# FanmingL/Recurrent-Offpolicy-RL

Hardware: AMD Instinct MI355X
Metric: env-steps/sec trained (higher is better)
Workload: dtype f32; 1 GPU; smamba_s32_c16_b2_nln SAC-REDQ update, B=64/GPU, T=1024, D=256 (configs[1]; N=8: configs[3]); row_length=1043, obs=17, act=6, critic=efc-8, global_rows=64, parallelism=dp1

## Files before the change

### include/resel_hip.h

```cpp
#ifndef RESEL_HIP_H
#define RESEL_HIP_H

#include <stddef.h>
#include <stdint.h>

#ifdef __cplusplus
extern "C" {
#endif

#define RESEL_OK 0
#define RESEL_EINVAL (-1)
#define RESEL_ELAUNCH (-2)

typedef void* resel_stream_t;

int resel_abi_version(void);
const char* resel_build_info(void);

enum {
    RESEL_PROF_SSCAN_FWD = 0, RESEL_PROF_SSCAN_BWD = 1, RESEL_PROF_ATTN_FWD = 2, RESEL_PROF_ATTN_DQ = 3, RESEL_PROF_ATTN_DKV = 4,
    RESEL_PROF_LINREC_REAL_FWD = 5, RESEL_PROF_LINREC_REAL_BWD = 6, RESEL_PROF_LINREC_COMPLEX_FWD = 7, RESEL_PROF_LINREC_COMPLEX_BWD = 8,
    RESEL_PROF_GRU_FWD = 9, RESEL_PROF_GRU_BWD = 10, RESEL_PROF_CONV_FWD = 11, RESEL_PROF_CONV_BWD = 12, RESEL_PROF_GEMM = 13,
    RESEL_PROF_SSCAN_FWD_LOCAL = 14, RESEL_PROF_SSCAN_BWD_LOCAL = 15,
    RESEL_PROF_NSLOTS = 16
};
int resel_profile_enable(int on);
int resel_profile_collect(int kernel_id, double* total_us, int* launches);

#define RESEL_SSCAN_CKPT 8
size_t resel_selective_scan_ckpt_bytes(int B, int L, int Di, int N);
size_t resel_selective_scan_fwd_workspace_bytes(int B, int L, int Di, int N, int time_segments);
int resel_selective_scan_fwd(const float* u, int64_t ld_u, const float* delta, int64_t ld_delta,
                             const float* z, int64_t ld_z, const float* A,
                             const float* Bm, int64_t ld_b, const float* Cm, int64_t ld_c,
                             const float* D, const float* delta_bias, const float* start,
                             float* out, int64_t ld_out, float* ckpt, float* last_state, void* workspace,
                             int B, int L, int Di, int N, int delta_softplus, int time_segments,
                             void* amax_out, unsigned amax_epoch, resel_stream_t stream);

size_t resel_selective_scan_bwd_workspace_bytes(int B, int L, int Di, int N, int time_segments);
int resel_selective_scan_bwd(const float* u, int64_t ld_u, const float* delta, int64_t ld_delta,
                             const float* z, int64_t ld_z, const float* A,
                             const float* Bm, int64_t ld_b, const float* Cm, int64_t ld_c,
                             const float* D, const float* delta_bias, const float* start,
                             const float* dout, int64_t ld_dout, const float* ckpt,
                             float* du, int64_t ld_du, float* ddelta, int64_t ld_ddelta, float* dz, int64_t ld_dz,
                             float* dBm, int64_t ld_db, float* dCm, int64_t ld_dc,
                             float* dA, float* dD, float* ddelta_bias, void* workspace,
                             int B, int L, int Di, int N, int delta_softplus, int time_segments,
                             void* amax_dz, void* amax_ddelta, unsigned amax_epoch, resel_stream_t stream);

int resel_causal_conv1d_fwd(const float* x, int64_t ld_x, const float* w, const float* bias, const float* mask,
                            float* y, int64_t ld_y, int B, int L, int Di, int K, int silu, void* amax_y, unsigned amax_epoch,
                            resel_stream_t stream);
size_t resel_causal_conv1d_bwd_workspace_bytes(int B, int L, int Di, int K);
int resel_causal_conv1d_bwd(const float* x, int64_t ld_x, const float* w, const float* bias, const float* mask,
                            const float* dy, int64_t ld_dy, float* dx, int64_t ld_dx, float* dw, float* dbias,
                            void* workspace, int B, int L, int Di, int K, int silu, void* amax_dx, unsigned amax_epoch,
                            resel_stream_t stream);
int resel_causal_conv1d_bwd2(const float* x, int64_t ld_x, const float* w, const float* bias, const float* mask,
                             const float* dy, int64_t ld_dy, const float* dy2, int64_t ld_dy2, float* dx, int64_t ld_dx,
                             float* dw, float* dbias, void* workspace, int B, int L, int Di, int K, int silu,
                             void* amax_dx, unsigned amax_epoch, resel_stream_t stream);

int resel_add_layernorm_fwd(const float* x, const float* residual, const float* w, const float* b,
                            float* y, float* res_out, float* stats, int M, int C, float eps, int rms, int act,
                            void* amax_y, unsigned amax_epoch, resel_stream_t stream);
size_t resel_add_layernorm_bwd_workspace_bytes(int M, int C);
int resel_add_layernorm_bwd(const float* dy, const float* dres_in, const float* res, const float* w, const float* b,
                            const float* stats, float* dx, float* dw, float* db, void* workspace,
                            int M, int C, int rms, int has_bias, int act, void* amax_dx, unsigned amax_epoch, resel_stream_t stream);

int resel_linrec_real_fwd(const float* v, const float* f, int64_t ld_u, const float* start, const float* h0, float* h,
                          int B, int L, int C, int fuse_act, void* amax_h, unsigned amax_epoch, resel_stream_t stream);
int resel_linrec_real_bwd(const float* v, const float* f, int64_t ld_u, const float* start, const float* h0, const float* h,
                          const float* dh, float* dv, float* df, int64_t ld_du, int B, int L, int C, int fuse_act,
                          void* amax_du, unsigned amax_epoch, resel_stream_t stream);
int resel_linrec_complex_fwd(const float* vr, const float* vi, int64_t ld_u, const float* lam_re, const float* lam_im,
                             const float* gamma, const float* start, const float* h0r, const float* h0i,
                             float* hr, float* hi, int B, int L, int C, void* amax_h, unsigned amax_epoch, resel_stream_t stream);
size_t resel_linrec_complex_bwd_workspace_bytes(int B, int L, int C);
int resel_linrec_complex_bwd(const float* vr, const float* vi, int64_t ld_u, const float* lam_re, const float* lam_im,
                             const float* gamma, const float* start, const float* h0r, const float* h0i,
// ... 184 lines not shown
```

### recurrent-offpolicy-rl_amd/csrc/resel_common.h

```cpp
#pragma once
#include <hip/hip_runtime.h>
#include <hip/hip_ext.h>
#include <stdint.h>
#include "../../include/resel_hip.h"

#define RESEL_LOG2E 1.4426950408889634f
#define RESEL_LN2 0.6931471805599453f

namespace resel {

typedef const float __attribute__((address_space(4)))* cfloat_p;
__device__ __forceinline__ cfloat_p as_uniform(const float* p) {
    return (cfloat_p)(uintptr_t)p;
}

__device__ __forceinline__ float fast_exp2(float x) { return __builtin_amdgcn_exp2f(x); }
__device__ __forceinline__ float fast_exp(float x) { return __builtin_amdgcn_exp2f(x * RESEL_LOG2E); }
__device__ __forceinline__ float fast_rcp(float x) { return __builtin_amdgcn_rcpf(x); }

__device__ __forceinline__ float sigmoidf_(float x) { return fast_rcp(1.0f + fast_exp(-x)); }
__device__ __forceinline__ float siluf_(float x) { return x * fast_rcp(1.0f + fast_exp(-x)); }
__device__ __forceinline__ float dsiluf_(float x) {
    float s = sigmoidf_(x);
    return s * (1.0f + x * (1.0f - s));
// ... 73 lines not shown
    (void)hipEventCreate(&b);
    hipExtLaunchKernelGGL(kernel, grid, block, lds, s, a, b, 0, args...);
    prof_push(slot, a, b);
}

#define RESEL_AMAX_SUBSLOTS 8
#define RESEL_AMAX_STRIDE 16
struct AmaxOut { unsigned long long* slot; unsigned epoch; };
__device__ __forceinline__ float amax4(float m, float4 v) {
    return fmaxf(fmaxf(m, fmaxf(__builtin_fabsf(v.x), __builtin_fabsf(v.y))), fmaxf(__builtin_fabsf(v.z), __builtin_fabsf(v.w)));
}
__device__ __forceinline__ void amax_publish_wave(float m, AmaxOut o) {
    if (o.slot == nullptr) return;
#pragma unroll
    for (int s = 32; s > 0; s >>= 1) m = fmaxf(m, __shfl_xor(m, s, 64));
    if (__lane_id() == 0) {
        unsigned long long* w = o.slot + RESEL_AMAX_STRIDE * ((blockIdx.x + blockIdx.y + blockIdx.z) & (RESEL_AMAX_SUBSLOTS - 1));
        const unsigned long long mine = ((unsigned long long)o.epoch << 32) | __float_as_uint(m);
        if (*(volatile unsigned long long*)w < mine) atomicMax(w, mine);
    }
}
__device__ __forceinline__ float amax_read(const float* handle) {
    const unsigned long long* h = reinterpret_cast<const unsigned long long*>(handle);
    const int j = __lane_id() & (RESEL_AMAX_SUBSLOTS - 1);
    unsigned long long v = h[RESEL_AMAX_STRIDE * j];
#pragma unroll
    for (int s = RESEL_AMAX_SUBSLOTS / 2; s > 0; s >>= 1) {
        const unsigned long long o = __shfl_xor(v, s, 64);
        v = o > v ? o : v;
    }
    return __uint_as_float((unsigned)(v & 0xffffffffu));
}

inline int launch_status() { return hipGetLastError() == hipSuccess ? RESEL_OK : RESEL_ELAUNCH; }
const unsigned long long* dropout_offset_base();
inline bool aligned16(const void* p) { return (reinterpret_cast<uintptr_t>(p) & 15u) == 0; }

}
```

### recurrent-offpolicy-rl_amd/csrc/selective_scan.hip

```cpp
#include "resel_common.h"
#include <hip/hip_ext.h>
#include <type_traits>
#include <vector>

namespace {
using namespace resel;

template <typename K, typename P>
void launch_maybe_timed(int slot, K kernel, dim3 grid, dim3 block, hipStream_t s, const P& p) {
    launch_timed(slot, kernel, grid, block, 0, s, p);
}
#ifdef SSCAN_STAMP
unsigned long long* g_stamps = nullptr;
#endif

constexpr int TILE_C = 64;
constexpr int CKS = RESEL_SSCAN_CKPT;
constexpr int SC = 16;
constexpr int SCH = 8;
static_assert(2 * CKS == SC && CKS == SCH, "a backward sub-chunk is two checkpoint intervals: each 8-step half starts from a stored state");

struct FwdParams {
    const float *u, *delta, *z, *A, *Bm, *Cm, *D, *delta_bias, *start;
    float *out, *ckpt, *last_state;
// ... 1035 lines not shown
                                        const float* Bm, int64_t ld_b, const float* Cm, int64_t ld_c,
                                        const float* D, const float* delta_bias, const float* start,
                                        float* out, int64_t ld_out, float* ckpt, float* last_state, void* workspace,
                                        int B, int L, int Di, int N, int delta_softplus, int time_segments,
                                        void* amax_out, unsigned amax_epoch, resel_stream_t stream) {
    if (!u || !delta || !A || !Bm || !Cm || !out || B <= 0 || L <= 0 || Di <= 0) return RESEL_EINVAL;
    if (amax_out && (reinterpret_cast<uintptr_t>(amax_out) & 7u)) return RESEL_EINVAL;
    if (Di % 4 != 0 || ld_u % 4 || ld_delta % 4 || ld_out % 4 || (z && ld_z % 4)) return RESEL_EINVAL;
    if (!aligned16(u) || !aligned16(delta) || !aligned16(out) || (z && !aligned16(z))) return RESEL_EINVAL;
    if ((D && !aligned16(D)) || (delta_bias && !aligned16(delta_bias))) return RESEL_EINVAL;
    FwdParams p{u, delta, z, A, Bm, Cm, D, delta_bias, start, out, ckpt, last_state,
                ld_u, ld_delta, ld_z, ld_b, ld_c, ld_out, B, L, Di, N, n_ckpt(L), delta_softplus & 3,
                (Di + TILE_C - 1) / TILE_C,
                (ld_b % 4 == 0 && ld_c % 4 == 0 && aligned16(Bm) && aligned16(Cm)) ? 1 : 0, (delta_softplus >> 2) & 1, 0, 1, nullptr, nullptr,
                AmaxOut{(unsigned long long*)amax_out, amax_epoch}};
#ifdef SSCAN_STAMP
    p.stamps = g_stamps;
#endif
    hipStream_t s = (hipStream_t)stream;
    switch (N) {
        case 4: return launch_fwd<1, 4, 32>(p, time_segments, workspace, s);
        case 8: return launch_fwd<2, 4, 32>(p, time_segments, workspace, s);
        case 16: return launch_fwd<4, 4, 32>(p, time_segments, workspace, s);
        case 32: return launch_fwd<8, 4, 32>(p, time_segments, workspace, s);
        case 64: return launch_fwd<8, 8, 32>(p, time_segments, workspace, s);
        default: return RESEL_EINVAL;
    }
}

extern "C" size_t resel_selective_scan_bwd_workspace_bytes(int B, int L, int Di, int N, int time_segments) {
    return bwd_ws(B, L, Di, N, time_segments).total;
}

extern "C" int resel_selective_scan_bwd(const float* u, int64_t ld_u, const float* delta, int64_t ld_delta,
                                        const float* z, int64_t ld_z, const float* A,
                                        const float* Bm, int64_t ld_b, const float* Cm, int64_t ld_c,
                                        const float* D, const float* delta_bias, const float* start,
                                        const float* dout, int64_t ld_dout, const float* ckpt,
                                        float* du, int64_t ld_du, float* ddelta, int64_t ld_ddelta,
                                        float* dz, int64_t ld_dz, float* dBm, int64_t ld_db, float* dCm, int64_t ld_dc,
                                        float* dA, float* dD, float* ddelta_bias, void* workspace,
                                        int B, int L, int Di, int N, int delta_softplus, int time_segments,
                                        void* amax_dz, void* amax_ddelta, unsigned amax_epoch, resel_stream_t stream) {
    if (!u || !delta || !A || !Bm || !Cm || !dout || !du || !ddelta || !dBm || !dCm || !dA || !workspace)
        return RESEL_EINVAL;
    if ((reinterpret_cast<uintptr_t>(amax_dz) & 7u) || (reinterpret_cast<uintptr_t>(amax_ddelta) & 7u)) return RESEL_EINVAL;
    if (B <= 0 || L <= 0 || Di <= 0 || Di % 4 != 0 || N % 4 != 0) return RESEL_EINVAL;
    if ((z != nullptr) != (dz != nullptr)) return RESEL_EINVAL;
    if (n_ckpt(L) > 0 && !ckpt) return RESEL_EINVAL;
    if (ld_u % 4 || ld_delta % 4 || ld_dout % 4 || ld_du % 4 || ld_ddelta % 4 || (z && (ld_z % 4 || ld_dz % 4)))
        return RESEL_EINVAL;
    if (!aligned16(u) || !aligned16(delta) || !aligned16(dout) || !aligned16(du) || !aligned16(ddelta) ||
        (z && (!aligned16(z) || !aligned16(dz))) || (D && !aligned16(D)) || (delta_bias && !aligned16(delta_bias)) ||
        !aligned16(workspace))
        return RESEL_EINVAL;
    const BwdWs ws = bwd_ws(B, L, Di, N, time_segments);
    char* base = (char*)workspace;
    BwdParams p{u, delta, z, A, Bm, Cm, D, delta_bias, start, dout, ckpt, du, ddelta, dz,
                (float*)(base + ws.dB), (float*)(base + ws.dC), (float*)(base + ws.dA), (float*)(base + ws.dD),
                (float*)(base + ws.dbias),
                ld_u, ld_delta, ld_z, ld_b, ld_c, ld_dout, ld_du, ld_ddelta, ld_dz,
                B, L, Di, N, n_ckpt(L), delta_softplus & 3, (Di + TILE_C - 1) / TILE_C,
                (ld_b % 4 == 0 && ld_c % 4 == 0 && aligned16(Bm) && aligned16(Cm)) ? 1 : 0, (delta_softplus >> 2) & 1,
                ws.nseg > 1 ? ((L + ws.nseg - 1) / ws.nseg + 31) / 32 * 32 : L, ws.nseg,
                ws.nseg > 1 ? (float*)(base + ws.carry) : nullptr, ws.nseg > 1 ? (float*)(base + ws.sdl) : nullptr,
                AmaxOut{(unsigned long long*)amax_dz, amax_epoch}, AmaxOut{(unsigned long long*)amax_ddelta, amax_epoch}};
    hipStream_t s = (hipStream_t)stream;
    int rc;
    switch (N) {
        case 4: rc = launch_bwd<1, 4>(p, s); break;
        case 8: rc = launch_bwd<2, 4>(p, s); break;
        case 16: rc = launch_bwd<4, 4>(p, s); break;
        case 32: rc = launch_bwd<8, 4>(p, s); break;
        case 64: rc = launch_bwd<8, 8>(p, s); break;
        default: return RESEL_EINVAL;
    }
    if (rc != RESEL_OK) return rc;
    const int64_t ntok = (int64_t)B * L;
    const int64_t n4 = ntok * (N / 4);
    hipLaunchKernelGGL(sscan_reduce_bc_kernel, dim3((unsigned)((n4 + 255) / 256), 2), dim3(256), 0, s,
                       p.dB_part, p.dC_part, p.nd, ntok, N, dBm, ld_db, dCm, ld_dc);
    const int64_t na = (int64_t)Di * N;
    hipLaunchKernelGGL(sscan_param_grads_kernel, dim3((unsigned)((na + 15) / 16), 3), dim3(256), 0, s,
                       p.dA_part, p.dD_part, p.dbias_part, B * ws.nseg, (int)na, Di, A, p.a_log, dA, dD, ddelta_bias);
    return launch_status();
}
```

### recurrent-offpolicy-rl_amd/csrc/skinny_gemm.hip

```cpp
#include "resel_common.h"

namespace {
using namespace resel;

typedef float f32x16 __attribute__((ext_vector_type(16)));

__device__ __forceinline__ int acc_row(int r, int half) { return (r >> 2) * 8 + half * 4 + (r & 3); }

template <int NT>
__global__ __launch_bounds__(256) void atb_kernel(const float* __restrict__ Wm, int64_t ldw, int Wd, const float* __restrict__ Nm,
                                                  int64_t ldn, int Nd, float* __restrict__ part, int64_t K, int rows_per,
                                                  int transposed) {
    const int lane = threadIdx.x & 63, wave = threadIdx.x >> 6;
    const int half = lane >> 5, col = lane & 31;
    const int wb = blockIdx.y * 512 + wave * 128;
    if (wb >= Wd) return;
    const int64_t k0 = (int64_t)blockIdx.x * rows_per;
    const int64_t k1 = k0 + rows_per < K ? k0 + rows_per : K;
    f32x16 acc[4][NT];
#pragma unroll
    for (int e = 0; e < 4; ++e)
#pragma unroll
        for (int t = 0; t < NT; ++t)
#pragma unroll
// ... 16 lines not shown
            for (int t = 0; t < NT; ++t) b[u][t] = (ok && n_ok[t]) ? Nm[kr * ldn + 32 * t + col] : 0.f;
        }
#pragma unroll
        for (int u = 0; u < UN; ++u)
#pragma unroll
            for (int t = 0; t < NT; ++t) {
                acc[0][t] = __builtin_amdgcn_mfma_f32_32x32x2f32(a[u].x, b[u][t], acc[0][t], 0, 0, 0);
                acc[1][t] = __builtin_amdgcn_mfma_f32_32x32x2f32(a[u].y, b[u][t], acc[1][t], 0, 0, 0);
                acc[2][t] = __builtin_amdgcn_mfma_f32_32x32x2f32(a[u].z, b[u][t], acc[2][t], 0, 0, 0);
                acc[3][t] = __builtin_amdgcn_mfma_f32_32x32x2f32(a[u].w, b[u][t], acc[3][t], 0, 0, 0);
            }
    }
    float* dst = part + (int64_t)blockIdx.x * Wd * Nd;
#pragma unroll
    for (int e = 0; e < 4; ++e)
#pragma unroll
        for (int t = 0; t < NT; ++t) {
            const int n = 32 * t + col;
            if (n >= Nd) continue;
#pragma unroll
            for (int r = 0; r < 16; ++r) {
                const int w = wb + 4 * acc_row(r, half) + e;
                if (w < Wd) dst[transposed ? (int64_t)n * Wd + w : (int64_t)w * Nd + n] = acc[e][t][r];
            }
        }
}

inline int pick_ksplit(int64_t K, int Wd, int Nd) {
    int64_t ks = (int64_t)(16 << 20) / ((int64_t)Wd * Nd * 4);
    if (ks > 512) ks = 512;
    if (ks < 32) ks = 32;
    if (ks > (K + 1) / 2) ks = (K + 1) / 2;
    return (int)(ks < 1 ? 1 : ks);
}

}

extern "C" {

size_t resel_atb_workspace_bytes(int64_t K, int Wd, int Nd) {
    return (size_t)pick_ksplit(K, Wd, Nd) * Wd * Nd * sizeof(float);
}

int resel_atb(const float* wide, int64_t ldw, int Wd, const float* narrow, int64_t ldn, int Nd, float* out, int transposed,
              void* workspace, int64_t K, resel_stream_t stream) {
    if (!wide || !narrow || !out || !workspace || K <= 0 || Wd <= 0 || Nd <= 0) return RESEL_EINVAL;
    if (Nd > 96 || (Wd & 3) || (ldw & 3) || !aligned16(wide)) return RESEL_EINVAL;
    const int ks = pick_ksplit(K, Wd, Nd);
    int rows_per = (int)((K + ks - 1) / ks);
    rows_per += rows_per & 1;
    const int nsplit = (int)((K + rows_per - 1) / rows_per);
    const dim3 grid(nsplit, (Wd + 511) / 512), block(256);
    hipStream_t s = (hipStream_t)stream;
    float* part = (float*)workspace;
    const int NT = (Nd + 31) / 32;
    switch (NT) {
        case 1: hipLaunchKernelGGL(atb_kernel<1>, grid, block, 0, s, wide, ldw, Wd, narrow, ldn, Nd, part, K, rows_per, transposed); break;
        case 2: hipLaunchKernelGGL(atb_kernel<2>, grid, block, 0, s, wide, ldw, Wd, narrow, ldn, Nd, part, K, rows_per, transposed); break;
        default: hipLaunchKernelGGL(atb_kernel<3>, grid, block, 0, s, wide, ldw, Wd, narrow, ldn, Nd, part, K, rows_per, transposed); break;
    }
    launch_colsum(part, (int64_t)Wd * Nd, nsplit, Wd * Nd, out, s);
    return launch_status();
}

}
```

### recurrent-offpolicy-rl_amd/offpolicy_rnn/hip/_lib.py

```python
import ctypes
import os
from ctypes import c_float, c_int, c_int64, c_size_t, c_uint64, c_void_p

_HERE = os.path.dirname(os.path.abspath(__file__))
LIB_PATH = os.environ.get('RESEL_HIP_LIBRARY') or os.path.join(_HERE, 'libresel_hip.so')
ABI_VERSION = 11
_lib = None

P, I, L, F, S, U = c_void_p, c_int, c_int64, c_float, c_void_p, c_uint64
E = ctypes.c_uint

RESET_MAX_SEGS, RESET_MAX_COUNTERS = 16, 8


class ResetSeg(ctypes.Structure):
    _fields_ = [('base', c_void_p), ('row_stride', c_int64), ('width', ctypes.c_int32)]


class ResetSegs(ctypes.Structure):
    _fields_ = [('seg', ResetSeg * RESET_MAX_SEGS)]


class ResetCounters(ctypes.Structure):
    _fields_ = [('pos', c_void_p * RESET_MAX_COUNTERS)]


SIGNATURES = {
    'resel_abi_version': (c_int, []),
    'resel_build_info': (ctypes.c_char_p, []),
    'resel_profile_enable': (c_int, [I]),
    'resel_profile_collect': (c_int, [I, P, P]),
    'resel_selective_scan_ckpt_bytes': (c_size_t, [I, I, I, I]),
    'resel_selective_scan_fwd_workspace_bytes': (c_size_t, [I, I, I, I, I]),
    'resel_selective_scan_fwd': (c_int, [P, L, P, L, P, L, P, P, L, P, L, P, P, P, P, L, P, P, P, I, I, I, I, I, I, P, E, S]),
    'resel_selective_scan_bwd_workspace_bytes': (c_size_t, [I, I, I, I, I]),
    'resel_selective_scan_bwd': (c_int, [P, L, P, L, P, L, P, P, L, P, L, P, P, P, P, L, P,
                                         P, L, P, L, P, L, P, L, P, L, P, P, P, P, I, I, I, I, I, I, P, P, E, S]),
    'resel_causal_conv1d_fwd': (c_int, [P, L, P, P, P, P, L, I, I, I, I, I, P, E, S]),
    'resel_causal_conv1d_bwd_workspace_bytes': (c_size_t, [I, I, I, I]),
    'resel_causal_conv1d_bwd': (c_int, [P, L, P, P, P, P, L, P, L, P, P, P, I, I, I, I, I, P, E, S]),
    'resel_causal_conv1d_bwd2': (c_int, [P, L, P, P, P, P, L, P, L, P, L, P, P, P, I, I, I, I, I, P, E, S]),
    'resel_add_layernorm_fwd': (c_int, [P, P, P, P, P, P, P, I, I, F, I, I, P, E, S]),
    'resel_add_layernorm_bwd_workspace_bytes': (c_size_t, [I, I]),
    'resel_add_layernorm_bwd': (c_int, [P, P, P, P, P, P, P, P, P, P, I, I, I, I, I, P, E, S]),
    'resel_linrec_real_fwd': (c_int, [P, P, L, P, P, P, I, I, I, I, P, E, S]),
    'resel_linrec_real_bwd': (c_int, [P, P, L, P, P, P, P, P, P, L, I, I, I, I, P, E, S]),
    'resel_linrec_complex_fwd': (c_int, [P, P, L, P, P, P, P, P, P, P, P, I, I, I, P, E, S]),
    'resel_linrec_complex_bwd_workspace_bytes': (c_size_t, [I, I, I]),
    'resel_place_blocks': (c_int, [P, L, I, I, I, P, P, P, P, P, P, S]),
    'resel_lru_params_fwd': (c_int, [P, P, I, S]),
    'resel_lru_params_bwd': (c_int, [P, P, P, I, S]),
    'resel_linrec_complex_bwd': (c_int, [P, P, L, P, P, P, P, P, P, P, P, P, P, P, P, L, P, P, P, P, I, I, I, S]),
    'resel_gru_workspace_bytes': (c_size_t, [I, I, I]),
    'resel_gru_seq_fwd': (c_int, [P, P, P, P, P, P, P, I, I, I, S]),
    'resel_gru_seq_bwd': (c_int, [P, P, P, P, P, P, P, P, I, I, I, S]),
    'resel_gru_multi_workspace_bytes': (c_size_t, [I, I, I, I]),
    'resel_gru_multi_fwd': (c_int, [I, P, P, P, P, P, P, P, I, I, I, S]),
    'resel_gru_multi_form': (c_int, [I, I, I]),
    'resel_attn_varlen_fwd_workspace_bytes': (c_size_t, [I, I]),
    'resel_attn_varlen_fwd': (c_int, [P, P, P, P, P, P, I, I, I, I, I, F, F, U, U, S]),
    'resel_attn_varlen_bwd_workspace_bytes': (c_size_t, [I, I, I, I, I]),
    'resel_attn_varlen_bwd': (c_int, [P, P, P, P, P, P, P, P, I, I, I, I, I, F, F, U, U, S]),
    'resel_attn_varlen_fwd_padded': (c_int, [P, P, P, P, P, P, I, I, I, I, I, F, F, U, U, S]),
    'resel_attn_varlen_bwd_padded': (c_int, [P, P, P, P, P, P, P, P, I, I, I, I, I, F, F, U, U, S]),
    'resel_pack_rows': (c_int, [P, L, P, P, P, L, I, I, S]),
    'resel_unpack_rows': (c_int, [P, L, P, P, P, L, I, I, I, S]),
    'resel_dropout': (c_int, [P, P, L, F, U, U, S]),
    'resel_dropout_offset_base': (c_int, [P]),
    'resel_gelu_dropout_fwd': (c_int, [P, P, L, F, U, U, P, E, S]),
    'resel_gelu_dropout_bwd': (c_int, [P, P, P, L, F, U, U, P, E, S]),
# ... 82 lines not shown
```

### recurrent-offpolicy-rl_amd/offpolicy_rnn/hip/ops.py

```python
import ctypes
import os
from typing import Optional

import torch

from ._lib import check, lib


def _need_cuda(name, *ts):
    for t in ts:
        if t is not None and not t.is_cuda:
            raise RuntimeError(f'RESeL-HIP: {name} needs CUDA tensors (got a {t.device} tensor); the HIP kernels are the '
                               f'only implementation of this op - there is no CPU fallback.')


def _p(t: Optional[torch.Tensor]):
    return None if t is None else ctypes.c_void_p(t.data_ptr())


if hasattr(torch._C, '_cuda_getCurrentRawStream') and hasattr(torch._C, '_cuda_getDevice'):
    def _stream():
        return ctypes.c_void_p(torch._C._cuda_getCurrentRawStream(torch._C._cuda_getDevice()))
else:
    def _stream():
# ... 38 lines not shown
    out = {}
    for kid, name in enumerate(PROF_SLOTS):
        tot, n = ctypes.c_double(0.0), ctypes.c_int(0)
        check(lib().resel_profile_collect(kid, ctypes.byref(tot), ctypes.byref(n)), 'profile_collect')
        if n.value:
            out[name] = (n.value, tot.value / n.value)
    return out


SSCAN_TIME_SEGMENTS = int(os.environ.get('RESEL_SSCAN_TIME_SEGMENTS', '0'))


def _sscan_fwd(Bsz, L, u, delta, z, A, Bm, Cm, D, delta_bias, start, out, ck, last, softplus, amax_out=None, epoch=0):
    Di, N = A.shape
    nb = lib().resel_selective_scan_fwd_workspace_bytes(Bsz, L, Di, N, SSCAN_TIME_SEGMENTS)
    check(lib().resel_selective_scan_fwd(
        _p(u), u.stride(-2), _p(delta), delta.stride(-2), _p(z), 0 if z is None else z.stride(-2), _p(A),
        _p(Bm), Bm.stride(-2), _p(Cm), Cm.stride(-2), _p(D), _p(delta_bias), _p(start),
        _p(out), out.stride(-2), _p(ck), _p(last), _p(_ws(nb, u.device) if nb else None), Bsz, L, Di, N, softplus,
        SSCAN_TIME_SEGMENTS, amax_out, epoch, _stream()), 'selective_scan_fwd')


def _sscan_bwd(Bsz, L, u, delta, z, A, Bm, Cm, D, delta_bias, start, dout, ck, du, ddelta, dz, dB, dC, dA, dD, dbias, softplus,
               amax_dz=None, amax_ddelta=None, epoch=0):
    Di, N = A.shape
    ws = _ws(lib().resel_selective_scan_bwd_workspace_bytes(Bsz, L, Di, N, SSCAN_TIME_SEGMENTS), u.device)
    check(lib().resel_selective_scan_bwd(
        _p(u), u.stride(-2), _p(delta), delta.stride(-2), _p(z), 0 if z is None else z.stride(-2), _p(A),
        _p(Bm), Bm.stride(-2), _p(Cm), Cm.stride(-2), _p(D), _p(delta_bias), _p(start),
        _p(dout), dout.stride(-2), _p(ck),
        _p(du), du.stride(-2), _p(ddelta), ddelta.stride(-2), _p(dz), 0 if dz is None else dz.stride(-2),
        _p(dB), dB.stride(-2), _p(dC), dC.stride(-2), _p(dA), _p(dD), _p(dbias), _p(ws),
        Bsz, L, Di, N, softplus, SSCAN_TIME_SEGMENTS, amax_dz, amax_ddelta, epoch, _stream()), 'selective_scan_bwd')


def _conv_fwd(Bsz, L, x, w, bias, mask, y, act, amax_y=None, epoch=0):
    Di, K = w.shape
    check(lib().resel_causal_conv1d_fwd(_p(x), x.stride(-2), _p(w), _p(bias), _p(mask), _p(y), y.stride(-2), Bsz, L, Di, K, act,
                                        amax_y, epoch, _stream()), 'causal_conv1d_fwd')


def _conv_bwd(Bsz, L, x, w, bias, mask, dy, dy2, dx, dw, db, act, amax_dx=None, epoch=0):
    Di, K = w.shape
    ws = _ws(lib().resel_causal_conv1d_bwd_workspace_bytes(Bsz, L, Di, K), x.device)
    check(lib().resel_causal_conv1d_bwd2(_p(x), x.stride(-2), _p(w), _p(bias), _p(mask), _p(dy), dy.stride(-2),
                                         _p(dy2), 0 if dy2 is None else dy2.stride(-2), _p(dx), dx.stride(-2), _p(dw), _p(db), _p(ws),
                                         Bsz, L, Di, K, act, amax_dx, epoch, _stream()), 'causal_conv1d_bwd')


class SelectiveScanFn(torch.autograd.Function):

    @staticmethod
    def forward(ctx, u, delta, A, Bm, Cm, D, z, delta_bias, start, delta_softplus, return_last_state):
        _need_cuda('selective_scan', u, delta, A, Bm, Cm)
        u, delta, Bm, Cm = _tok_major(u), _tok_major(delta), _tok_major(Bm), _tok_major(Cm)
        z = None if z is None else _tok_major(z)
        A = A.float().contiguous()
        D = None if D is None else D.float().contiguous()
        delta_bias = None if delta_bias is None else delta_bias.float().contiguous()
        Bsz, L, Di = u.shape
        N = A.shape[1]
        start = _flags(start, Bsz, L)
        out = torch.empty(Bsz, L, Di, dtype=torch.float32, device=u.device)
        need_grad = any(ctx.needs_input_grad)
        ck = None
        if need_grad:
# ... 73 lines not shown
        need_grad = any(ctx.needs_input_grad)
        ck = _ws(lib().resel_selective_scan_ckpt_bytes(Bsz, L, Di, N), x.device) if need_grad else None
        y = torch.empty(M, Di, dtype=torch.float32, device=x.device)
        h_y, p_y, e_y = _slot_args(track, x.device)
        _sscan_fwd(Bsz, L, xc, dt, xz[:, Di:], A, x_dbl[:, R:R + N], x_dbl[:, R + N:], D, None, startf, y, ck, None, 6, p_y, e_y)
        tag_amax(y, h_y)
        out = mm_nt(y, out_w)
        ctx.handles = keep_handles(ctx.ax, h_xc, h_y)
        ctx.save_for_backward(x2, in_w, cw, conv_b, xproj_w, dt_w, dt_b, A, D, out_w, maskf, startf, xz, xc, x_dbl, dt, y, ck)
        ctx.dims = (Bsz, L, Dm, Di, N, R, K, conv_w.shape)
        return out.view(Bsz, L, -1)

    @staticmethod
    def backward(ctx, dout):
        (x2, in_w, cw, conv_b, xproj_w, dt_w, dt_b, A, D, out_w, maskf, startf, xz, xc, x_dbl, dt, y, ck) = ctx.saved_tensors
        Bsz, L, Dm, Di, N, R, K, cw_shape = ctx.dims
        M = Bsz * L
        dev = x2.device
        do2 = dout.reshape(M, -1)
        if not do2.is_contiguous():
            do2 = do2.contiguous()
        ax, h_xc, h_y = live_handles(ctx.handles)
        d_out_w = wgrad(do2, y, amax_x=h_y)
        dy = mm_nn(do2, out_w)
        dxz = torch.empty(M, 2 * Di, dtype=torch.float32, device=dev)
        dx_dbl = torch.empty(M, R + 2 * N, dtype=torch.float32, device=dev)
        dxc = torch.empty(M, Di, dtype=torch.float32, device=dev)
        ddt = torch.empty(M, Di, dtype=torch.float32, device=dev)
        dA = torch.empty(Di, N, dtype=torch.float32, device=dev)
        dD = torch.empty(Di, dtype=torch.float32, device=dev)
        ddt_b = torch.empty(Di, dtype=torch.float32, device=dev)
        track = amax_tracking() and M * Di >= (1 << 20)
        h_dxz, p_dxz, e_b = _slot_args(track, dev)
        h_ddt, p_ddt, _ = _slot_args(track, dev)
        _sscan_bwd(Bsz, L, xc, dt, xz[:, Di:], A, x_dbl[:, R:R + N], x_dbl[:, R + N:], D, None, startf, dy, ck,
                   dxc, ddt, dxz[:, Di:], dx_dbl[:, R:R + N], dx_dbl[:, R + N:], dA, dD, ddt_b, 6, p_dxz, p_ddt, e_b)
        tag_amax(ddt, h_ddt)
        d_dt_w = atb(ddt, x_dbl[:, :R]) if R <= 32 and Di % 4 == 0 and ddt.stride(1) == 1 and ddt.stride(0) % 4 == 0 \
            else gemm_f32(ddt, x_dbl[:, :R], False, False)
        mm_nn(ddt, dt_w, out=dx_dbl[:, :R])
        d_xproj_w = wgrad(dx_dbl, xc, amax_x=h_xc)
        gx = mm_nn(dx_dbl, xproj_w)
        dcw = torch.empty(Di, K, dtype=torch.float32, device=dev)
        dcb = torch.empty(Di, dtype=torch.float32, device=dev) if conv_b is not None else None
        _conv_bwd(Bsz, L, xz, cw, conv_b, maskf, dxc, gx, dxz, dcw, dcb, 1, p_dxz, e_b)
        tag_amax(dxz, h_dxz)
        d_in_w = wgrad(dxz, x2, amax_x=ax)
        dx = mm_nn(dxz, in_w).view(Bsz, L, Dm) if ctx.needs_input_grad[0] else None
        return (dx, d_in_w, dcw.reshape(cw_shape), dcb, d_xproj_w, d_dt_w, ddt_b, dA, dD, d_out_w, None, None)


def mamba_inner_fn(x, in_w, conv_w, conv_b, xproj_w, dt_w, dt_b, A_log, D, out_w, mask=None, start=None):
    return MambaInnerFn.apply(x.float().contiguous(), in_w, conv_w, conv_b, xproj_w, dt_w, dt_b, A_log, D, out_w, mask, start)


class CausalConv1dFn(torch.autograd.Function):
    @staticmethod
    def forward(ctx, x, weight, bias, mask, activation):
        _need_cuda('causal_conv1d', x, weight)
        x = _tok_major(x)
        Bsz, L, Di = x.shape
        w = weight.float().reshape(Di, -1).contiguous()
        bias = None if bias is None else bias.float().contiguous()
        mask = _flags(mask, Bsz, L)
        y = torch.empty(Bsz, L, Di, dtype=torch.float32, device=x.device)
        _conv_fwd(Bsz, L, x, w, bias, mask, y, int(bool(activation)))
        ctx.save_for_backward(x, w, bias, mask)
        ctx.act = bool(activation)
        ctx.wshape = weight.shape
        return y

    @staticmethod
    def backward(ctx, dy):
# ... 1517 lines not shown
```

Before: 3.049 million env-steps/s.

## Fuse dB/dC reduction, dt_proj weight grad and input grad into one scan-bwd tail kernel

Replaces the separate dB/dC partial-reduction kernel, the atb weight-gradient GEMM and the mm_nn input-gradient GEMM after the selective-scan backward with a single MFMA kernel. Each block reads ddelta once and computes both d_dt_w partials and dx_dr, then a colsum reduces the partials. This removes extra passes over ddelta and several kernel launches. In exchange it drops amax tracking of ddelta on this path and adds a small workspace for the partials.

```diff
diff --git a/include/resel_hip.h b/include/resel_hip.h
--- a/include/resel_hip.h
+++ b/include/resel_hip.h
@@ -49,6 +49,19 @@
                              float* dA, float* dD, float* ddelta_bias, void* workspace,
                              int B, int L, int Di, int N, int delta_softplus, int time_segments,
                              void* amax_dz, void* amax_ddelta, unsigned amax_epoch, resel_stream_t stream);
+
+int resel_selective_scan_bwd_narrow(const float* u, int64_t ld_u, const float* delta, int64_t ld_delta,
+                                    const float* z, int64_t ld_z, const float* A,
+                                    const float* Bm, int64_t ld_b, const float* Cm, int64_t ld_c,
+                                    const float* D, const float* delta_bias, const float* start,
+                                    const float* dout, int64_t ld_dout, const float* ckpt,
+                                    float* du, int64_t ld_du, float* ddelta, int64_t ld_ddelta, float* dz, int64_t ld_dz,
+                                    float* dBm, int64_t ld_db, float* dCm, int64_t ld_dc,
+                                    float* dA, float* dD, float* ddelta_bias, void* workspace,
+                                    int B, int L, int Di, int N, int delta_softplus, int time_segments,
+                                    void* amax_dz, void* amax_ddelta, unsigned amax_epoch,
+                                    const float* dt_w, int R, const float* x_dr, int64_t ld_x, float* dx_dr, int64_t ld_dx,
+                                    float* d_dt_w, void* narrow_workspace, resel_stream_t stream);
 
 int resel_causal_conv1d_fwd(const float* x, int64_t ld_x, const float* w, const float* bias, const float* mask,
                             float* y, int64_t ld_y, int B, int L, int Di, int K, int silu, void* amax_y, unsigned amax_epoch,
diff --git a/recurrent-offpolicy-rl_amd/csrc/resel_common.h b/recurrent-offpolicy-rl_amd/csrc/resel_common.h
--- a/recurrent-offpolicy-rl_amd/csrc/resel_common.h
+++ b/recurrent-offpolicy-rl_amd/csrc/resel_common.h
@@ -129,6 +129,11 @@
     return __uint_as_float((unsigned)(v & 0xffffffffu));
 }
 
+bool mixer_bwd_narrow_ok(int Di, int R, int N, int64_t ld_ddelta, int64_t ld_x, int64_t ld_dx);
+void launch_mixer_bwd_narrow(const float* ddelta, int64_t ld_ddelta, int Di, const float* x_dr, int64_t ld_x, int R, const float* dt_w,
+                             const float* partB, const float* partC, int nd, int N, float* dB, int64_t ld_db, float* dC, int64_t ld_dc,
+                             float* dx_dr, int64_t ld_dx, float* d_dt_w, void* workspace, int64_t ntok, hipStream_t s);
+
 inline int launch_status() { return hipGetLastError() == hipSuccess ? RESEL_OK : RESEL_ELAUNCH; }
 const unsigned long long* dropout_offset_base();
 inline bool aligned16(const void* p) { return (reinterpret_cast<uintptr_t>(p) & 15u) == 0; }
diff --git a/recurrent-offpolicy-rl_amd/csrc/selective_scan.hip b/recurrent-offpolicy-rl_amd/csrc/selective_scan.hip
--- a/recurrent-offpolicy-rl_amd/csrc/selective_scan.hip
+++ b/recurrent-offpolicy-rl_amd/csrc/selective_scan.hip
@@ -1091,16 +1091,18 @@
     return bwd_ws(B, L, Di, N, time_segments).total;
 }
 
-extern "C" int resel_selective_scan_bwd(const float* u, int64_t ld_u, const float* delta, int64_t ld_delta,
-                                        const float* z, int64_t ld_z, const float* A,
-                                        const float* Bm, int64_t ld_b, const float* Cm, int64_t ld_c,
-                                        const float* D, const float* delta_bias, const float* start,
-                                        const float* dout, int64_t ld_dout, const float* ckpt,
-                                        float* du, int64_t ld_du, float* ddelta, int64_t ld_ddelta,
-                                        float* dz, int64_t ld_dz, float* dBm, int64_t ld_db, float* dCm, int64_t ld_dc,
-                                        float* dA, float* dD, float* ddelta_bias, void* workspace,
-                                        int B, int L, int Di, int N, int delta_softplus, int time_segments,
-                                        void* amax_dz, void* amax_ddelta, unsigned amax_epoch, resel_stream_t stream) {
+struct NarrowTail { const float* dt_w; const float* x_dr; int64_t ld_x; float* dx_dr; int64_t ld_dx; float* d_dt_w; void* ws; int R; };
+
+static int scan_bwd(const float* u, int64_t ld_u, const float* delta, int64_t ld_delta,
+                    const float* z, int64_t ld_z, const float* A,
+                    const float* Bm, int64_t ld_b, const float* Cm, int64_t ld_c,
+                    const float* D, const float* delta_bias, const float* start,
+                    const float* dout, int64_t ld_dout, const float* ckpt,
+                    float* du, int64_t ld_du, float* ddelta, int64_t ld_ddelta,
+                    float* dz, int64_t ld_dz, float* dBm, int64_t ld_db, float* dCm, int64_t ld_dc,
+                    float* dA, float* dD, float* ddelta_bias, void* workspace,
+                    int B, int L, int Di, int N, int delta_softplus, int time_segments,
+                    void* amax_dz, void* amax_ddelta, unsigned amax_epoch, resel_stream_t stream, const NarrowTail* tail) {
     if (!u || !delta || !A || !Bm || !Cm || !dout || !du || !ddelta || !dBm || !dCm || !dA || !workspace)
         return RESEL_EINVAL;
     if ((reinterpret_cast<uintptr_t>(amax_dz) & 7u) || (reinterpret_cast<uintptr_t>(amax_ddelta) & 7u)) return RESEL_EINVAL;
@@ -1137,10 +1139,49 @@
     if (rc != RESEL_OK) return rc;
     const int64_t ntok = (int64_t)B * L;
     const int64_t n4 = ntok * (N / 4);
-    hipLaunchKernelGGL(sscan_reduce_bc_kernel, dim3((unsigned)((n4 + 255) / 256), 2), dim3(256), 0, s,
-                       p.dB_part, p.dC_part, p.nd, ntok, N, dBm, ld_db, dCm, ld_dc);
+    if (tail)
+        launch_mixer_bwd_narrow(ddelta, ld_ddelta, Di, tail->x_dr, tail->ld_x, tail->R, tail->dt_w, p.dB_part, p.dC_part, p.nd, N,
+                                dBm, ld_db, dCm, ld_dc, tail->dx_dr, tail->ld_dx, tail->d_dt_w, tail->ws, ntok, s);
+    else
+        hipLaunchKernelGGL(sscan_reduce_bc_kernel, dim3((unsigned)((n4 + 255) / 256), 2), dim3(256), 0, s,
+                           p.dB_part, p.dC_part, p.nd, ntok, N, dBm, ld_db, dCm, ld_dc);
     const int64_t na = (int64_t)Di * N;
     hipLaunchKernelGGL(sscan_param_grads_kernel, dim3((unsigned)((na + 15) / 16), 3), dim3(256), 0, s,
                        p.dA_part, p.dD_part, p.dbias_part, B * ws.nseg, (int)na, Di, A, p.a_log, dA, dD, ddelta_bias);
     return launch_status();
 }
+
+extern "C" int resel_selective_scan_bwd(const float* u, int64_t ld_u, const float* delta, int64_t ld_delta,
+                                        const float* z, int64_t ld_z, const float* A,
+                                        const float* Bm, int64_t ld_b, const float* Cm, int64_t ld_c,
+                                        const float* D, const float* delta_bias, const float* start,
+                                        const float* dout, int64_t ld_dout, const float* ckpt,
+                                        float* du, int64_t ld_du, float* ddelta, int64_t ld_ddelta,
+                                        float* dz, int64_t ld_dz, float* dBm, int64_t ld_db, float* dCm, int64_t ld_dc,
+                                        float* dA, float* dD, float* ddelta_bias, void* workspace,
+                                        int B, int L, int Di, int N, int delta_softplus, int time_segments,
+                                        void* amax_dz, void* amax_ddelta, unsigned amax_epoch, resel_stream_t stream) {
+    return scan_bwd(u, ld_u, delta, ld_delta, z, ld_z, A, Bm, ld_b, Cm, ld_c, D, delta_bias, start, dout, ld_dout, ckpt, du, ld_du,
+                    ddelta, ld_ddelta, dz, ld_dz, dBm, ld_db, dCm, ld_dc, dA, dD, ddelta_bias, workspace, B, L, Di, N, delta_softplus,
+                    time_segments, amax_dz, amax_ddelta, amax_epoch, stream, nullptr);
+}
+
+extern "C" int resel_selective_scan_bwd_narrow(const float* u, int64_t ld_u, const float* delta, int64_t ld_delta,
+                                               const float* z, int64_t ld_z, const float* A,
+                                               const float* Bm, int64_t ld_b, const float* Cm, int64_t ld_c,
+                                               const float* D, const float* delta_bias, const float* start,
+                                               const float* dout, int64_t ld_dout, const float* ckpt,
+                                               float* du, int64_t ld_du, float* ddelta, int64_t ld_ddelta,
+                                               float* dz, int64_t ld_dz, float* dBm, int64_t ld_db, float* dCm, int64_t ld_dc,
+                                               float* dA, float* dD, float* ddelta_bias, void* workspace,
+                                               int B, int L, int Di, int N, int delta_softplus, int time_segments,
+                                               void* amax_dz, void* amax_ddelta, unsigned amax_epoch,
+                                               const float* dt_w, int R, const float* x_dr, int64_t ld_x, float* dx_dr, int64_t ld_dx,
+                                               float* d_dt_w, void* narrow_workspace, resel_stream_t stream) {
+    if (!dt_w || !x_dr || !dx_dr || !d_dt_w || !narrow_workspace) return RESEL_EINVAL;
+    if (!mixer_bwd_narrow_ok(Di, R, N, ld_ddelta, ld_x, ld_dx) || ld_x < R || ld_dx < R) return RESEL_EINVAL;
+    const NarrowTail tail{dt_w, x_dr, ld_x, dx_dr, ld_dx, d_dt_w, narrow_workspace, R};
+    return scan_bwd(u, ld_u, delta, ld_delta, z, ld_z, A, Bm, ld_b, Cm, ld_c, D, delta_bias, start, dout, ld_dout, ckpt, du, ld_du,
+                    ddelta, ld_ddelta, dz, ld_dz, dBm, ld_db, dCm, ld_dc, dA, dD, ddelta_bias, workspace, B, L, Di, N, delta_softplus,
+                    time_segments, amax_dz, amax_ddelta, amax_epoch, stream, &tail);
+}
diff --git a/recurrent-offpolicy-rl_amd/csrc/skinny_gemm.hip b/recurrent-offpolicy-rl_amd/csrc/skinny_gemm.hip
--- a/recurrent-offpolicy-rl_amd/csrc/skinny_gemm.hip
+++ b/recurrent-offpolicy-rl_amd/csrc/skinny_gemm.hip
@@ -72,6 +72,180 @@
     if (ks < 32) ks = 32;
     if (ks > (K + 1) / 2) ks = (K + 1) / 2;
     return (int)(ks < 1 ? 1 : ks);
+}
+
+typedef float f32x4 __attribute__((ext_vector_type(4)));
+constexpr int NB_TOK = 16;
+constexpr int NB_LD = 68;
+constexpr int NB_MAX_R = 16, NB_MAX_DI = 512;
+
+template <int QW>
+__global__ __launch_bounds__(256) void mixer_bwd_narrow_kernel(const float* __restrict__ ddt, int64_t ldd, int Di,
+                                                               const float* __restrict__ xr, int64_t ldx, int R,
+                                                               const float* __restrict__ dtw, const float* __restrict__ partB,
+                                                               const float* __restrict__ partC, int nd, int N, float* outB, int64_t ldB,
+                                                               float* outC, int64_t ldC, float* dxr, int64_t ldo,
+                                                               float* __restrict__ part, int64_t M, int rows_per) {
+    __shared__ __attribute__((aligned(16))) float s_t[4][NB_TOK * NB_LD];
+    __shared__ float s_r[2][4][NB_TOK][17];
+    const int tid = threadIdx.x, lane = tid & 63, wave = tid >> 6;
+    const int i = lane & 15, j = lane >> 4;
+    const int64_t k0 = (int64_t)blockIdx.x * rows_per;
+    const int64_t k1 = k0 + rows_per < M ? k0 + rows_per : M;
+
+    {
+        const int n4 = N / 4;
+        const int cnt = (int)(k1 - k0) * n4;
+        for (int idx = tid; idx < 2 * cnt; idx += 256) {
+            const int which = idx >= cnt;
+            const int q = which ? idx - cnt : idx;
+            const float* ps = which ? partC : partB;
+            const int64_t tok = k0 + q / n4;
+            const int c = (q % n4) * 4;
+            float4 acc = make_float4(0.f, 0.f, 0.f, 0.f);
+            for (int t0 = 0; t0 < nd; t0 += 8) {
+                float4 v[8];
+#pragma unroll
+                for (int t = 0; t < 8; ++t) v[t] = ld4(ps + ((int64_t)(t0 + t < nd ? t0 + t : nd - 1) * M + tok) * N + c);
+#pragma unroll
+                for (int t = 0; t < 8; ++t)
+                    if (t0 + t < nd) { acc.x += v[t].x; acc.y += v[t].y; acc.z += v[t].z; acc.w += v[t].w; }
+            }
+            float* o = (which ? outC + tok * ldC : outB + tok * ldB) + c;
+            o[0] = acc.x; o[1] = acc.y; o[2] = acc.z; o[3] = acc.w;
+        }
+    }
+
+    float w[QW][4][4];
+    f32x4 accw[QW][4];
+#pragma unroll
+    for (int q = 0; q < QW; ++q) {
+        const int cb = (wave + 4 * q) * 64;
+#pragma unroll
+        for (int s = 0; s < 4; ++s)
+#pragma unroll
+            for (int e = 0; e < 4; ++e) {
+                const int c = cb + 4 * (j + 4 * s) + e;
+                w[q][s][e] = (c < Di && i < R) ? dtw[(int64_t)c * R + i] : 0.f;
+            }
+#pragma unroll
+        for (int e = 0; e < 4; ++e) accw[q][e] = f32x4{0.f, 0.f, 0.f, 0.f};
+    }
+
+    float4 nxt[QW][4];
+    float nx[4];
+    auto fetch = [&](int64_t t0) {
+#pragma unroll
+        for (int u = 0; u < 4; ++u) {
+            const int64_t tok = t0 + 4 * u + j;
+            const bool ok = tok < k1;
+            const int64_t tk = ok ? tok : k1 - 1;
+            const float xv = xr[tk * ldx + (i < R ? i : 0)];
+            nx[u] = (ok && i < R) ? xv : 0.f;
+#pragma unroll
+            for (int q = 0; q < QW; ++q) {
+                const int c = (wave + 4 * q) * 64 + 4 * i;
+                const float4 v = ld4(ddt + tk * ldd + (c < Di ? c : 0));
+                nxt[q][u] = (ok && c < Di) ? v : make_float4(0.f, 0.f, 0.f, 0.f);
+            }
+        }
+    };
+    fetch(k0);
+    float* st = s_t[wave];
+    int par = 0;
+    for (int64_t t0 = k0; t0 < k1; t0 += NB_TOK, par ^= 1) {
+        float4 a[QW][4];
+        float xb[4];
+#pragma unroll
+        for (int u = 0; u < 4; ++u) {
+            xb[u] = nx[u];
+#pragma unroll
+            for (int q = 0; q < QW; ++q) a[q][u] = nxt[q][u];
+        }
+        if (t0 + NB_TOK < k1) fetch(t0 + NB_TOK);
+        f32x4 accx[4];
+#pragma unroll
+        for (int e = 0; e < 4; ++e) accx[e] = f32x4{0.f, 0.f, 0.f, 0.f};
+#pragma unroll
+        for (int q = 0; q < QW; ++q) {
+#pragma unroll
+            for (int u = 0; u < 4; ++u) {
+                accw[q][0] = __builtin_amdgcn_mfma_f32_16x16x4f32(a[q][u].x, xb[u], accw[q][0], 0, 0, 0);
+                accw[q][1] = __builtin_amdgcn_mfma_f32_16x16x4f32(a[q][u].y, xb[u], accw[q][1], 0, 0, 0);
+                accw[q][2] = __builtin_amdgcn_mfma_f32_16x16x4f32(a[q][u].z, xb[u], accw[q][2], 0, 0, 0);
+                accw[q][3] = __builtin_amdgcn_mfma_f32_16x16x4f32(a[q][u].w, xb[u], accw[q][3], 0, 0, 0);
+                st4(st + (4 * u + j) * NB_LD + 4 * i, a[q][u]);
+            }
+            __builtin_amdgcn_fence(__ATOMIC_RELEASE, "wavefront");
+            __builtin_amdgcn_wave_barrier();
+            __builtin_amdgcn_fence(__ATOMIC_ACQUIRE, "wavefront");
+            float4 v[4];
+#pragma unroll
+            for (int s = 0; s < 4; ++s) v[s] = ld4(st + i * NB_LD + 4 * (j + 4 * s));
+            __builtin_amdgcn_fence(__ATOMIC_RELEASE, "wavefront");
+            __builtin_amdgcn_wave_barrier();
+            __builtin_amdgcn_fence(__ATOMIC_ACQUIRE, "wavefront");
+#pragma unroll
+            for (int s = 0; s < 4; ++s) {
+                accx[0] = __builtin_amdgcn_mfma_f32_16x16x4f32(v[s].x, w[q][s][0], accx[0], 0, 0, 0);
+                accx[1] = __builtin_amdgcn_mfma_f32_16x16x4f32(v[s].y, w[q][s][1], accx[1], 0, 0, 0);
+                accx[2] = __builtin_amdgcn_mfma_f32_16x16x4f32(v[s].z, w[q][s][2], accx[2], 0, 0, 0);
+                accx[3] = __builtin_amdgcn_mfma_f32_16x16x4f32(v[s].w, w[q][s][3], accx[3], 0, 0, 0);
+            }
+        }
+#pragma unroll
+        for (int r = 0; r < 4; ++r) s_r[par][wave][4 * j + r][i] = (accx[0][r] + accx[1][r]) + (accx[2][r] + accx[3][r]);
+        __syncthreads();
+        {
+            const int row = tid >> 4, col = tid & 15;
+            const float sum = ((s_r[par][0][row][col] + s_r[par][1][row][col]) + s_r[par][2][row][col]) + s_r[par][3][row][col];
+            if (t0 + row < k1 && col < R) dxr[(t0 + row) * ldo + col] = sum;
+        }
+    }
+
+    float* dst = part + (int64_t)blockIdx.x * Di * R;
+    if (i < R) {
+#pragma unroll
+        for (int q = 0; q < QW; ++q)
+#pragma unroll
+            for (int e = 0; e < 4; ++e)
+#pragma unroll
+                for (int r = 0; r < 4; ++r) {
+                    const int c = (wave + 4 * q) * 64 + 4 * (4 * j + r) + e;
+                    if (c < Di) dst[(int64_t)c * R + i] = accw[q][e][r];
+                }
+    }
+}
+
+inline int narrow_rows_per(int64_t M, int Di, int R) {
+    const int ks = pick_ksplit(M, Di, R);
+    int64_t rp = ((M + ks - 1) / ks + NB_TOK - 1) / NB_TOK * NB_TOK;
+    if (rp < 4 * NB_TOK) rp = 4 * NB_TOK;
+    return (int)rp;
+}
+
+}
+
+namespace resel {
+
+bool mixer_bwd_narrow_ok(int Di, int R, int N, int64_t ld_ddelta, int64_t ld_x, int64_t ld_dx) {
+    return R >= 1 && R <= NB_MAX_R && Di >= 4 && Di <= NB_MAX_DI && Di % 4 == 0 && N % 4 == 0 && ld_ddelta % 4 == 0 && ld_x % 4 == 0 &&
+           ld_dx % 4 == 0;
+}
+
+void launch_mixer_bwd_narrow(const float* ddelta, int64_t ld_ddelta, int Di, const float* x_dr, int64_t ld_x, int R, const float* dt_w,
+                             const float* partB, const float* partC, int nd, int N, float* dB, int64_t ld_db, float* dC, int64_t ld_dc,
+                             float* dx_dr, int64_t ld_dx, float* d_dt_w, void* workspace, int64_t ntok, hipStream_t s) {
+    const int rows_per = narrow_rows_per(ntok, Di, R);
+    const int nblk = (int)((ntok + rows_per - 1) / rows_per);
+    float* part = (float*)workspace;
+    if (Di <= 256)
+        hipLaunchKernelGGL(mixer_bwd_narrow_kernel<1>, dim3(nblk), dim3(256), 0, s, ddelta, ld_ddelta, Di, x_dr, ld_x, R, dt_w, partB, partC,
+                           nd, N, dB, ld_db, dC, ld_dc, dx_dr, ld_dx, part, ntok, rows_per);
+    else
+        hipLaunchKernelGGL(mixer_bwd_narrow_kernel<2>, dim3(nblk), dim3(256), 0, s, ddelta, ld_ddelta, Di, x_dr, ld_x, R, dt_w, partB, partC,
+                           nd, N, dB, ld_db, dC, ld_dc, dx_dr, ld_dx, part, ntok, rows_per);
+    launch_colsum(part, (int64_t)Di * R, nblk, Di * R, d_dt_w, s);
 }
 
 }
diff --git a/recurrent-offpolicy-rl_amd/offpolicy_rnn/hip/_lib.py b/recurrent-offpolicy-rl_amd/offpolicy_rnn/hip/_lib.py
--- a/recurrent-offpolicy-rl_amd/offpolicy_rnn/hip/_lib.py
+++ b/recurrent-offpolicy-rl_amd/offpolicy_rnn/hip/_lib.py
@@ -36,6 +36,9 @@
     'resel_selective_scan_bwd_workspace_bytes': (c_size_t, [I, I, I, I, I]),
     'resel_selective_scan_bwd': (c_int, [P, L, P, L, P, L, P, P, L, P, L, P, P, P, P, L, P,
                                          P, L, P, L, P, L, P, L, P, L, P, P, P, P, I, I, I, I, I, I, P, P, E, S]),
+    'resel_selective_scan_bwd_narrow': (c_int, [P, L, P, L, P, L, P, P, L, P, L, P, P, P, P, L, P,
+                                                P, L, P, L, P, L, P, L, P, L, P, P, P, P, I, I, I, I, I, I, P, P, E,
+                                                P, I, P, L, P, L, P, P, S]),
     'resel_causal_conv1d_fwd': (c_int, [P, L, P, P, P, P, L, I, I, I, I, I, P, E, S]),
     'resel_causal_conv1d_bwd_workspace_bytes': (c_size_t, [I, I, I, I]),
     'resel_causal_conv1d_bwd': (c_int, [P, L, P, P, P, P, L, P, L, P, P, P, I, I, I, I, I, P, E, S]),
diff --git a/recurrent-offpolicy-rl_amd/offpolicy_rnn/hip/ops.py b/recurrent-offpolicy-rl_amd/offpolicy_rnn/hip/ops.py
--- a/recurrent-offpolicy-rl_amd/offpolicy_rnn/hip/ops.py
+++ b/recurrent-offpolicy-rl_amd/offpolicy_rnn/hip/ops.py
@@ -94,6 +94,29 @@
         _p(du), du.stride(-2), _p(ddelta), ddelta.stride(-2), _p(dz), 0 if dz is None else dz.stride(-2),
         _p(dB), dB.stride(-2), _p(dC), dC.stride(-2), _p(dA), _p(dD), _p(dbias), _p(ws),
         Bsz, L, Di, N, softplus, SSCAN_TIME_SEGMENTS, amax_dz, amax_ddelta, epoch, _stream()), 'selective_scan_bwd')
+
+
+def _narrow_tail_ok(ddt, x_dr, dx_dr, dt_w):
+    Di, R = dt_w.shape
+    return (R <= 16 and Di <= 512 and Di % 4 == 0 and ddt.stride(1) == 1 and ddt.stride(0) % 4 == 0
+            and x_dr.stride(1) == 1 and x_dr.stride(0) % 4 == 0 and dx_dr.stride(1) == 1 and dx_dr.stride(0) % 4 == 0
+            and dt_w.is_contiguous() and dt_w.dtype == torch.float32)
+
+
+def _sscan_bwd_narrow(Bsz, L, u, delta, z, A, Bm, Cm, D, delta_bias, start, dout, ck, du, ddelta, dz, dB, dC, dA, dD, dbias, softplus,
+                      dt_w, x_dr, dx_dr, d_dt_w, amax_dz=None, epoch=0):
+    Di, N = A.shape
+    R = dt_w.shape[1]
+    ws = _ws(lib().resel_selective_scan_bwd_workspace_bytes(Bsz, L, Di, N, SSCAN_TIME_SEGMENTS), u.device)
+    nws = _ws(lib().resel_atb_workspace_bytes(Bsz * L, Di, R), u.device)
+    check(lib().resel_selective_scan_bwd_narrow(
+        _p(u), u.stride(-2), _p(delta), delta.stride(-2), _p(z), 0 if z is None else z.stride(-2), _p(A),
+        _p(Bm), Bm.stride(-2), _p(Cm), Cm.stride(-2), _p(D), _p(delta_bias), _p(start),
+        _p(dout), dout.stride(-2), _p(ck),
+        _p(du), du.stride(-2), _p(ddelta), ddelta.stride(-2), _p(dz), 0 if dz is None else dz.stride(-2),
+        _p(dB), dB.stride(-2), _p(dC), dC.stride(-2), _p(dA), _p(dD), _p(dbias), _p(ws),
+        Bsz, L, Di, N, softplus, SSCAN_TIME_SEGMENTS, amax_dz, None, epoch,
+        _p(dt_w), R, _p(x_dr), x_dr.stride(-2), _p(dx_dr), dx_dr.stride(-2), _p(d_dt_w), _p(nws), _stream()), 'selective_scan_bwd_narrow')
 
 
 def _conv_fwd(Bsz, L, x, w, bias, mask, y, act, amax_y=None, epoch=0):
@@ -233,13 +256,19 @@
         ddt_b = torch.empty(Di, dtype=torch.float32, device=dev)
         track = amax_tracking() and M * Di >= (1 << 20)
         h_dxz, p_dxz, e_b = _slot_args(track, dev)
-        h_ddt, p_ddt, _ = _slot_args(track, dev)
-        _sscan_bwd(Bsz, L, xc, dt, xz[:, Di:], A, x_dbl[:, R:R + N], x_dbl[:, R + N:], D, None, startf, dy, ck,
-                   dxc, ddt, dxz[:, Di:], dx_dbl[:, R:R + N], dx_dbl[:, R + N:], dA, dD, ddt_b, 6, p_dxz, p_ddt, e_b)
-        tag_amax(ddt, h_ddt)
-        d_dt_w = atb(ddt, x_dbl[:, :R]) if R <= 32 and Di % 4 == 0 and ddt.stride(1) == 1 and ddt.stride(0) % 4 == 0 \
-            else gemm_f32(ddt, x_dbl[:, :R], False, False)
-        mm_nn(ddt, dt_w, out=dx_dbl[:, :R])
+        if _narrow_tail_ok(ddt, x_dbl[:, :R], dx_dbl[:, :R], dt_w):
+            d_dt_w = torch.empty(Di, R, dtype=torch.float32, device=dev)
+            _sscan_bwd_narrow(Bsz, L, xc, dt, xz[:, Di:], A, x_dbl[:, R:R + N], x_dbl[:, R + N:], D, None, startf, dy, ck,
+                              dxc, ddt, dxz[:, Di:], dx_dbl[:, R:R + N], dx_dbl[:, R + N:], dA, dD, ddt_b, 6,
+                              dt_w, x_dbl[:, :R], dx_dbl[:, :R], d_dt_w, p_dxz, e_b)
+        else:
+            h_ddt, p_ddt, _ = _slot_args(track, dev)
+            _sscan_bwd(Bsz, L, xc, dt, xz[:, Di:], A, x_dbl[:, R:R + N], x_dbl[:, R + N:], D, None, startf, dy, ck,
+                       dxc, ddt, dxz[:, Di:], dx_dbl[:, R:R + N], dx_dbl[:, R + N:], dA, dD, ddt_b, 6, p_dxz, p_ddt, e_b)
+            tag_amax(ddt, h_ddt)
+            d_dt_w = atb(ddt, x_dbl[:, :R]) if R <= 32 and Di % 4 == 0 and ddt.stride(1) == 1 and ddt.stride(0) % 4 == 0 \
+                else gemm_f32(ddt, x_dbl[:, :R], False, False)
+            mm_nn(ddt, dt_w, out=dx_dbl[:, :R])
         d_xproj_w = wgrad(dx_dbl, xc, amax_x=h_xc)
         gx = mm_nn(dx_dbl, xproj_w)
         dcw = torch.empty(Di, K, dtype=torch.float32, device=dev)
```

New measurement: 3.071 million env-steps/s, median of 6. About the same (+0.7%).
